# superboubek/bcd

Hardware: AMD Instinct MI355X
Metric: Mpixels/sec denoised (3-scale, b=6, w=1) (higher is better)
Workload: dtype f32

## Files before the change

bcd_amd/csrc/bcd_api.hip:

```cpp
#include "bcd_ctx.h"

#include <algorithm>
#include <chrono>
#include <climits>
#include <cmath>
#include <cstdio>
#include <cstdlib>
#include <cstring>
#include <atomic>
#include <condition_variable>
#include <mutex>
#include <new>
#include <thread>
#include <string>
#include <utility>
#include <vector>

void set_err(bcd_hip_ctx *ctx, const std::string &msg)
{
    if (!ctx) return;
    std::lock_guard<std::mutex> lock(ctx->err_mutex);
    ctx->err = msg;
}

// ... 865 lines not shown
    if (!ctx) return BCD_HIP_EINVAL;
    ctx->profiling = enabled != 0;
    return BCD_HIP_OK;
}

int bcd_hip_set_concurrent_scales(bcd_hip_ctx *ctx, int enabled)
{
    if (!ctx) return BCD_HIP_EINVAL;
    ctx->concurrent_scales = enabled != 0;
    return BCD_HIP_OK;
}

int bcd_hip_set_strict_eigensolver(int enabled)
{
    bcd_bayes27_set_strict_eigensolver(enabled);
    return BCD_HIP_OK;
}

int bcd_hip_set_fast_similarity(bcd_hip_ctx *ctx, int enabled)
{
    if (!ctx) return BCD_HIP_EINVAL;
    ctx->fast_similarity = enabled != 0;
    return BCD_HIP_OK;
}

int bcd_hip_set_cu_share(bcd_hip_ctx *ctx, int percent)
{
    if (!ctx || percent < 1 || percent > 100) return BCD_HIP_EINVAL;
    ctx->cu_share_pct = percent;
    return BCD_HIP_OK;
// ... 892 lines not shown
```

bcd_amd/csrc/bcd_launch.h:

```cpp
#pragma once
#include "bcd_common.h"

#include <stddef.h>

size_t bcd_pairdist_lds_bytes(int D, int b);
hipError_t bcd_launch_pairdist(const float *hist, const float *ns, int W, int H, int D, int b, float *T, uint8_t *Cn, int fast, int *d_range_flag, float uni_n,
                               hipStream_t st);
hipError_t bcd_launch_uniform_n(const float *ns, int64_t npix, int *d_out, hipStream_t st);
hipError_t bcd_launch_compare_planes(const float *Ta, const uint8_t *Ca, const float *Tb, const uint8_t *Cb, int64_t n, unsigned long long *out, hipStream_t st);
hipError_t bcd_launch_selftest_div(uint32_t seed, int blocks, int per_thread, unsigned long long *d_mismatches, hipStream_t st);
hipError_t bcd_launch_masks(const float *T, const uint8_t *Cn, int W, int H, int w, int b, float tau, uint32_t *mask, int32_t *count, uint32_t *fwd_scratch,
                            hipStream_t st, const BcdBorderline *ap, const float *hist, const float *ns, int D);
hipError_t bcd_launch_masks_finish(int W, int H, int b, float tau, uint32_t *mask, int32_t *count, uint32_t *fwd_scratch, hipStream_t st, const BcdBorderline *ap,
                                   const float *hist, const float *ns, int D);
hipError_t bcd_launch_window_distances(const float *T, const uint8_t *Cn, int W, int H, int w, int b, int r, int c, float *out, hipStream_t st);

hipError_t bcd_launch_pairdist_moments(const float *colors, const float *pixcov, int W, int H, int b, float var_floor, float *T, uint8_t *Cn, hipStream_t st);

hipError_t bcd_pairdist_guide_launchable(int F, int has_var, int b);
hipError_t bcd_launch_pairdist_guide(const float *features, const float *variances, int F, const float *floors, int W, int H, int b, float *T, uint8_t *Cn,
                                     hipStream_t st);
hipError_t bcd_launch_gate_masks(uint32_t *mask, const uint32_t *gate, int32_t *nsim, int W, int H, int b, hipStream_t st);
hipError_t bcd_launch_scale_inplace(float *x, float a, int64_t n, hipStream_t st);

// ... 61 lines not shown

size_t bcd_bayes_lds_bytes(int w, int b);
size_t bcd_bayes_scratch_bytes_per_block(int w, int b);
hipError_t bcd_launch_bayes_strong(const float *colors, const float *pixcov, const uint32_t *mask, const int32_t *list, const int32_t *d_nlist, int *d_work, int blocks,
                                   int W, int H, int w, int b, float min_eig, float *sum, int32_t *cnt, float *gscratch, size_t gscratch_bytes, hipStream_t st);
hipError_t bcd_launch_bayes_weak(const float *colors, const uint32_t *mask, const int32_t *list, const int32_t *d_nlist, int blocks, int W, int H, int w, int b,
                                 float *sum, int32_t *cnt, hipStream_t st);
hipError_t bcd_launch_bayes_weak_tiles(const float *colors, const uint32_t *mask, const uint8_t *state, const int32_t *nsim, int min_strong, int W, int H, int b,
                                       float *sum, int32_t *cnt, hipStream_t st, int row_begin, int row_end, const long long *skip_if);
hipError_t bcd_launch_bayes_weak_tiles_layers(const BcdLayerTable &t, int layers, const uint32_t *mask, const uint8_t *state, const int32_t *nsim, int min_strong,
                                              int W, int H, int b, hipStream_t st, int row_begin, int row_end);

size_t bcd_bayes27_record_bytes();
void bcd_bayes27_set_strict_eigensolver(int on);
float bcd_bayes27_conv2(int strict);
hipError_t bcd_launch_jacobi27_batch(const float *A, int n, int *d_work, int blocks, float *eig, float *V, hipStream_t st, float conv2 = 1e-12f, float *Aout = nullptr,
                                     const int *d_n = nullptr, int first_item = 0);
hipError_t bcd_launch_bayes27(const float *colors, const float *pixcov, const uint32_t *mask, const int32_t *list, int first_item, int nb_items, int *d_work,
                              int num_cus, int W, int H, int b, float min_eig, float *records, float *sum, int32_t *cnt, int *d_spectral, hipStream_t st,
                              int defer_redo, const int *d_nb_items);
hipError_t bcd_launch_bayes27_redo(const float *colors, const float *pixcov, const uint32_t *mask, const int32_t *list, int first_item, int nb_items, int *d_work,
                                   int num_cus, int W, int H, int b, float min_eig, float *records, float *sum, int32_t *cnt, hipStream_t st);

size_t bcd_accum_snapshot_lds(int D);
hipError_t bcd_launch_accum_dense(const float *samples, const float *weights, int64_t p0, int64_t npix, int64_t N, int k, int channels, int nbins, float gamma,
                                  float maxval, float *st, hipStream_t s);
hipError_t bcd_launch_accum_dense_layers(const BcdAccumLayerIn &in, int nb_layers, const float *weights, int64_t p0, int64_t npix, int64_t N, int k, int channels,
                                         float *layers, hipStream_t s);
hipError_t bcd_launch_accum_segments_layers(const uint32_t *keys, const uint32_t *vals, int64_t n, int64_t N, const BcdAccumLayerIn &in, int nb_layers,
                                            const float *weights, float *layers, hipStream_t s);
// ... 23 lines not shown
```

bcd_amd/csrc/bcd_selftest.hip:

```cpp
#include "bcd_ctx.h"

#include <algorithm>
#include <cstring>

namespace {

struct DevAlloc {
    void *p = nullptr;
    DevAlloc() = default;
    DevAlloc(const DevAlloc &) = delete;
    DevAlloc &operator=(const DevAlloc &) = delete;
    ~DevAlloc() { if (p) (void)hipFree(p); }
};

}

extern "C" {

int bcd_hip_selftest_distance_kernels(bcd_hip_ctx *ctx, const float *d_hist, const float *d_ns, int W, int H, int D, int search_radius,
                                      int *variant, int64_t *mismatches)
{
    if (!ctx || !d_hist || !d_ns || !mismatches || W <= 0 || H <= 0 || D <= 0 || search_radius < 1) return bad(ctx, "bad argument");
    DEVICE_GUARD(ctx);
    touch(ctx->main);
// ... 142 lines not shown
    DEVICE_GUARD(ctx);
    touch(ctx->main);
    Work &wk = ctx->main;
    RCCHK(ensure(ctx, wk.counters, sizeof(Counters)));
    RCCHK(ensure(ctx, wk.work_q, BCD_WORK_INTS * sizeof(int32_t)));
    int32_t *d_c = (int32_t *)wk.work_q.p;
    HIPCHK(ctx, hipMemsetAsync(d_c, 0, BCD_WORK_INTS * sizeof(int32_t), wk.stream));
    HIPCHK(ctx, hipEventRecord(wk.ev_stage[0], wk.stream));
    HIPCHK(ctx, bcd_launch_jacobi27_batch(d_A, n, d_c, std::min(ctx->num_cus * 12, (n + 1) / 2), d_eig, d_V, wk.stream, bcd_bayes27_conv2(production_rule ? 0 : 1)));
    HIPCHK(ctx, hipEventRecord(wk.ev_stage[1], wk.stream));
    HIPCHK(ctx, hipStreamSynchronize(wk.stream));
    if (ms) *ms = stage_ms(wk, 0, 1);
    return BCD_HIP_OK;
}

int bcd_hip_selftest_division(bcd_hip_ctx *ctx, uint32_t seed, int64_t samples, int64_t *mismatches)
{
    if (!ctx || !mismatches || samples <= 0) return bad(ctx, "bad argument");
    DEVICE_GUARD(ctx);
    touch(ctx->main);
    RCCHK(ensure(ctx, ctx->main.counters, sizeof(Counters)));
    unsigned long long *d = &ctx->main.d_counters()->selftest.result;
    HIPCHK(ctx, hipMemsetAsync(d, 0, sizeof(unsigned long long), ctx->stream));
    const int per_thread = 1024, blocks = (int)std::min<int64_t>(1 << 20, (samples + 256ll * per_thread - 1) / (256ll * per_thread));
    HIPCHK(ctx, bcd_launch_selftest_div(seed, blocks, per_thread, d, ctx->stream));
    unsigned long long h = 0;
    HIPCHK(ctx, hipMemcpyAsync(&h, d, sizeof(h), hipMemcpyDeviceToHost, ctx->stream));
    HIPCHK(ctx, hipStreamSynchronize(ctx->stream));
    *mismatches = (int64_t)h;
    return BCD_HIP_OK;
// ... 117 lines not shown
```

bcd_amd/csrc/k_bayes27.hip:

```cpp
#include "bcd_common.h"
#include <atomic>
#include <cstdio>
#include <algorithm>
#include <cstdlib>

namespace {


constexpr int K = 27, KP = 28, LD = 29, P = 9, MSZ = KP * KP, CHUNK = MSZ / K;

typedef float v16f __attribute__((ext_vector_type(16)));

struct Geom27 {
    int W, H, b, side, words, maxS;
};

#define LDS_POINTER(p) __builtin_assume(__builtin_amdgcn_is_shared((const __attribute__((address_space(0))) void *)(p)))

__device__ inline float pos_phi(float di, float dj)
{
    const float hi = fmaxf(di, dj), lo = fminf(di, dj);
    if (lo > 0.f) return 1.f;
    if (hi <= 0.f) return 0.f;
    return hi * __builtin_amdgcn_rcpf(hi - lo);
// ... 392 lines not shown
            float out[JLD], vout[JLD];
#pragma unroll
            for (int k = 0; k < JLD; ++k) { out[YSTEP ? JSY[k] : JSX[k]] = row[k]; vout[YSTEP ? JSY[k] : JSX[k]] = vrow[k]; }
#pragma unroll
            for (int k = 0; k < JLD; ++k) vrow[k] = vout[k];
            if (isRow) {
#pragma unroll
                for (int q4 = 0; q4 < JLD / 4; ++q4)
                    reinterpret_cast<float4 *>(dst)[q4] = make_float4(out[4 * q4], out[4 * q4 + 1], out[4 * q4 + 2], out[4 * q4 + 3]);
            }
        }
        wave_sync();
        __builtin_amdgcn_sched_barrier(0);
}

__global__ __launch_bounds__(64, 3) void k_jacobi27_quads(const float *Ain, int n, int *work, float *__restrict__ eig,
                                                          float *__restrict__ Vout, float conv2, float *Aout, const int *d_n, int first_item)
{
    n = items_on_device(d_n, first_item, n);
    __shared__ float4 lds4[(2 * JQ_HALF + 32) / 4];
    float *lds = reinterpret_cast<float *>(lds4);
    int *place_tab = reinterpret_cast<int *>(lds + 2 * JQ_HALF);
    const int lane = threadIdx.x, h = lane >> 5, r = lane & 31;
    const bool isRow = r < KP;
    if (lane < KP) place_tab[lane] = JPLACE[lane];
    float *Ah = lds + h * JQ_HALF, *dv_h = Ah + JQ_MAT, *rot_h = dv_h + 32;
    const int rr_ = isRow ? r : JIDLE_ROW;
    const int sx = isRow ? JSX[rr_] : 0, sy = isRow ? JSY[rr_] : 0;
    float *src = Ah + JPLACE[rr_];
    float *dst_x = Ah + JPLACE[sx], *dst_y = Ah + JPLACE[sy];
    const float *wsrc = src + (isRow ? (r & ~3) : 0);
    const int me = r & 3;
    wave_sync();
    WorkCursor cursor = work_begin();
    for (;;) {
        const int pair = work_next(work, (n + 1) / 2, lane, cursor);
        if (pair < 0) break;
        const int first = 2 * pair;
        const int item = first + h;
        const bool live = item < n;
        {
            const float4 *gsrc = reinterpret_cast<const float4 *>(Ain + (size_t)(live ? item : first) * (KP * JLD));
            for (int e = r; e < KP * JLD / 4; e += 32) {
                float4 v = gsrc[e];
                const int e0 = 4 * e, rr = e0 / JLD, c0 = e0 - rr * JLD;
                if (!live) v = make_float4(rr == c0, rr == c0 + 1, rr == c0 + 2, rr == c0 + 3);
                *reinterpret_cast<float4 *>(Ah + place_tab[rr] + c0) = v;
            }
            if (isRow) dv_h[r] = 1.f;
        }
        wave_sync();
        float vrow[JLD];
// ... 48 lines not shown
            if (isRow) eig[(size_t)item * KP + r] = src[r];
        }
        if (Aout) {
            if (isRow) rot_h[r] = src[r];
            wave_sync();
            if (isRow && live) jacobi_write_correction(Aout + (size_t)item * (KP * JLD) + r * JLD, src, rot_h, r);
        }
        if (live) {
            if (r < K) {
                float4 *o = reinterpret_cast<float4 *>(Vout + (size_t)item * (KP * JLD) + r * JLD);
#pragma unroll
                for (int q4 = 0; q4 < JLD / 4; ++q4) o[q4] = make_float4(vrow[4 * q4], vrow[4 * q4 + 1], vrow[4 * q4 + 2], vrow[4 * q4 + 3]);
            }
        }
        wave_sync();
    }
}

__device__ void add_noise27(float *M, const float *noise, int lane, float sign)
{
    for (int t = lane; t < P * 9; t += 64) {
        int blk = t / 9, e = t - blk * 9, i = e / 3, j = e - i * 3;
        M[(3 * blk + i) * LD + 3 * blk + j] += sign * noise[blk * 6 + noise_idx(i, j)];
    }
    __syncthreads();
}


__device__ inline float bcast_lane(float v, int k) { return __int_as_float(__builtin_amdgcn_readlane(__float_as_int(v), k)); }

// ... 730 lines not shown
    for (int t = lane; t < P * 9; t += 64) {
        const int ro = t / 9, ij = t - 9 * ro, i = ij / 3, j = ij - 3 * i;
        float *e = tile + (3 * ro + i) * LD + 3 * ro + j;
        *e -= noise[ro * 6 + noise_idx(i, j)];
    }
    for (int e = lane; e < KP * (JLD / 4); e += 64) {
        const int r = e / (JLD / 4), q = e - r * (JLD / 4);
        const float *src = tile + r * LD + 4 * q;
        reinterpret_cast<float4 *>(recA)[e] = make_float4(src[0], src[1], src[2], src[3]);
    }
    const bool poisoned = noise_poisons_item(noise, lane);
    if (lane < P * 6) recX[lane] = noise[lane];
    if (lane < K) recX[P * 6 + lane] = poisoned ? __builtin_nanf("") : mean[lane];
}

template <int PHASE, int B = WB>
__global__ __launch_bounds__(64, PHASE == 1 ? 5 : 3) void k_bayes27w(const float *__restrict__ colors, const float *__restrict__ pixcov,
                                                 const uint32_t *__restrict__ mask, const int32_t *__restrict__ list,
                                                 int first_item, int nb_items, int *work, Geom27 g, float min_eig, Records27 rec, float *sum,
                                                 int32_t *cnt, const int *redo ,
                                                 const int *d_n = nullptr)
{
    extern __shared__ float lds[];
    const int lane = threadIdx.x;
    nb_items = items_on_device(d_n, first_item, nb_items);
    if (PHASE == 2 && redo) nb_items = redo[0];
    if (PHASE == 1 && redo && blockIdx.x == 0 && lane == 0) const_cast<int *>(redo)[0] = 0;
    float *Cm = lds, *A = Cm + MSZ, *V = A + MSZ, *Bm = V + MSZ;
    float *cwin = PHASE == 1 ? lds : Bm;
    static_assert(PHASE == 1 || B == WB, "the LDS finish (PHASE 2) exists for the default search radius only");
    float *nwin = cwin + W1L<B>::NWIN;
    float *cs = Bm + MSZ;
    float *noise = PHASE == 1 ? lds + W1L<B>::NOISE : cs + 2 * KP;
    float *mean = noise + 56;
    float *fl = mean + KP;
    uint16_t *mem = reinterpret_cast<uint16_t *>(PHASE == 1 ? lds + W1L<B>::MEM : fl + KP);
    static_assert(WPIX * 3 <= MSZ, "the colour window fits a matrix buffer");
    for (int e = lane; e < (PHASE == 1 ? W1L<B>::MEM_SLOTS : WinT<B>::MEM); e += 64) mem[e] = (uint16_t)((WinT<B>::AW + 1) * (PHASE == 1 ? 3 : 1));
    if (lane == 0) mean[K] = 0.f;
    __syncthreads();
    const int W = g.W, H = g.H;

  WorkCursor cursor = work_begin();
  for (;;) {
    int slot = work_next(work, nb_items, lane, cursor);
    if (slot < 0) break;
    if (PHASE == 2 && redo) slot = __builtin_amdgcn_readfirstlane(redo[1 + slot]);
    const int p = __builtin_amdgcn_readfirstlane(list[first_item + slot]);
    const int pr = p / W, pc = p - pr * W;
    float *recA = rec.A + (size_t)slot * MSZ, *recC = rec.C + (size_t)slot * MSZ, *recX = rec.aux + (size_t)slot * AUX27;

  if (PHASE == 1) {
    const int n = win_stage_phase1<B>(cwin, nwin, mem, colors, pixcov, mask, p, pr, pc, W, H, g.words, lane);
    win_noise_mean<B>(noise, mean, cwin, nwin, mem, n, lane, pixcov, (pr - (B + 1)) * W + pc - (B + 1), W);
    win_covariance<B>(nwin , cwin, mean, mem, n, lane);
    win_write_records(recA, recC, recX, nwin, noise, mean, lane);
    __syncthreads();
  } else {
    const int n = decode_members_win<WB>(mask, p, g.words, mem, lane);
    {
        const float *recV = rec.V + (size_t)slot * MSZ;
        for (int e = lane; e < MSZ / 4; e += 64) {
            reinterpret_cast<float4 *>(Cm)[e] = reinterpret_cast<const float4 *>(recC)[e];
            reinterpret_cast<float4 *>(V)[e] = reinterpret_cast<const float4 *>(recV)[e];
        }
        if (lane < P * 6) noise[lane] = recX[lane];
        if (lane < K) mean[lane] = recX[P * 6 + lane];
        if (lane < KP) fl[lane] = fmaxf(0.f, rec.eig[(size_t)slot * KP + lane]);
        __syncthreads();
    }
    pos_part_lds(Bm, A, fl, V, recA, rec.eig + (size_t)slot * KP, lane);
// ... 79 lines not shown
    {
        constexpr int row3 = WAW * 3;
        const long long base = (long long)p - (long long)(WB + 1) * W - (WB + 1);
        for (int e = lane; e < WAW * row3; e += 64) {
            int wy = e / row3, r = e - wy * row3, wx = r / 3;
            if (accC[wy * WAW + wx] != 0) unsafeAtomicAdd(sum + (base + (long long)wy * W) * 3 + r, accS[e]);
        }
        for (int e = lane; e < WPIX; e += 64) {
            int wy = e / WAW, wx = e - wy * WAW, c = accC[e];
            if (c != 0 && cnt) atomicAdd(cnt + (base + (long long)wy * W + wx), c);
        }
    }
    __syncthreads();
  }
  }
}

template <int B>
__global__ __launch_bounds__(64, 3) void k_finish27w(const float *__restrict__ colors, const uint32_t *__restrict__ mask,
                                                     const int32_t *__restrict__ list, int first_item, int nb_items, int *work, Geom27 g,
                                                     float min_eig, Records27 rec, float *sum, int32_t *cnt, int *redo ,
                                                     int *redo_total , const int *d_n)
{
    nb_items = items_on_device(d_n, first_item, nb_items);
    using G_ = WinT<B>;
    constexpr int AW = G_::AW, PIX = G_::PIX, GAP = G_::G;
    extern __shared__ float lds[];
    const int lane0 = threadIdx.x;
    float *cwin = lds, *accS = lds + G_::F2_ACCS;
    int *accC = reinterpret_cast<int *>(lds + G_::F2_ACCC);
// ... 197 lines not shown

hipError_t bcd_launch_jacobi27_batch(const float *A, int n, int *d_work, int blocks, float *eig, float *V, hipStream_t st, float conv2 = 1e-12f, float *Aout = nullptr,
                                     const int *d_n = nullptr, int first_item = 0);

static std::atomic<int> g_strict_eigen{ -1 };
void bcd_bayes27_set_strict_eigensolver(int on) { g_strict_eigen.store(on ? 1 : 0); }
static float jacobi_conv2()
{
    int v = g_strict_eigen.load();
    if (v < 0) { const char *e = getenv("BCD_HIP_STRICT_EIGEN"); v = (e && e[0] == '1') ? 1 : 0; g_strict_eigen.store(v); }
    return v ? JACOBI_CONV2_STRICT : JACOBI_CONV2_CORRECTED;
}

float bcd_bayes27_conv2(int strict) { return strict ? JACOBI_CONV2_STRICT : JACOBI_CONV2_CORRECTED; }

hipError_t bcd_launch_bayes27(const float *colors, const float *pixcov, const uint32_t *mask, const int32_t *list, int first_item, int nb_items,
                              int *d_work, int num_cus, int W, int H, int b, float min_eig, float *records, float *sum,
                              int32_t *cnt, int *d_spectral , hipStream_t st,
                              int defer_redo ,
                              const int *d_nb_items )
{
    const int *dn = d_nb_items;
    if (nb_items <= 0) return hipSuccess;
    Geom27 g;
    g.W = W; g.H = H; g.b = b; g.side = 2 * b + 1; g.words = (g.side * g.side + 31) / 32; g.maxS = g.side * g.side;
    if (g.words > 32) return hipErrorInvalidValue;
    Records27 rec;
    rec.A = records;
    rec.V = rec.A + (size_t)nb_items * MSZ;
    rec.C = rec.V + (size_t)nb_items * MSZ;
    rec.aux = rec.C + (size_t)nb_items * MSZ;
    rec.eig = rec.aux + (size_t)nb_items * AUX27;
    const size_t lds2 = bcd_bayes27_lds_bytes(b), lds1 = lds2 - 3 * MSZ * sizeof(float);
    const int per_cu1 = (int)std::min<size_t>(20, (size_t)160 * 1024 / lds1), per_cu2 = (int)std::min<size_t>(12, (size_t)160 * 1024 / lds2);
    if (b == WB) {
        const size_t wl1 = W1L<WB>::BYTES;
        const size_t wl2 = (size_t)W2_MEM * sizeof(float) + WMEM * sizeof(uint16_t);
        const int w_cu1 = (int)std::min<size_t>(20, (size_t)160 * 1024 / wl1), w_cu2 = (int)std::min<size_t>(12, (size_t)160 * 1024 / wl2);
        static const bool lds_algebra = [] { const char *e = getenv("BCD_HIP_FINISH_LDS"); return e && e[0] == '1'; }();
        int *redo = reinterpret_cast<int *>(rec.eig + (size_t)nb_items * KP);
        hipLaunchKernelGGL(k_bayes27w<1>, dim3(std::min(nb_items, num_cus * w_cu1)), dim3(64), wl1, st, colors, pixcov, mask, list, first_item, nb_items,
                           d_work, g, min_eig, rec, sum, cnt, lds_algebra ? nullptr : redo, dn);
        { hipError_t e = bcd_launch_jacobi27_batch(rec.A, nb_items, d_work + BCD_WORK_QUEUES * BCD_WORK_STRIDE, std::min((nb_items + 1) / 2, num_cus * 12), rec.eig, rec.V, st, jacobi_conv2(), rec.A, dn, first_item); if (e != hipSuccess) return e; }
        if (lds_algebra)
            hipLaunchKernelGGL(k_bayes27w<2>, dim3(std::min(nb_items, num_cus * w_cu2)), dim3(64), wl2, st, colors, pixcov, mask, list, first_item, nb_items,
                               d_work + 2 * BCD_WORK_QUEUES * BCD_WORK_STRIDE, g, min_eig, rec, sum, cnt, nullptr, dn);
        else {
            const size_t wl3 = WinT<WB>::F2_BYTES;
            hipLaunchKernelGGL(k_finish27w<WB>, dim3(std::min(nb_items, num_cus * 12)), dim3(64), wl3, st, colors, mask, list, first_item, nb_items,
                               d_work + 2 * BCD_WORK_QUEUES * BCD_WORK_STRIDE, g, min_eig, rec, sum, cnt, redo, d_spectral, dn);
            if (!defer_redo)
                hipLaunchKernelGGL(k_bayes27w<2>, dim3(std::min(nb_items, num_cus * 2)), dim3(64), wl2, st, colors, pixcov, mask, list, first_item, nb_items,
                                   d_work + 3 * BCD_WORK_QUEUES * BCD_WORK_STRIDE, g, min_eig, rec, sum, cnt, redo, dn);
        }
        return hipGetLastError();
    }
    constexpr int WB2 = 12;
    static const bool finish_lds_b12 = [] { const char *e = getenv("BCD_HIP_FINISH_LDS"); return e && e[0] == '1'; }();
// ... 55 lines not shown
    const size_t wl2 = (size_t)W2_MEM * sizeof(float) + WMEM * sizeof(uint16_t);
    hipLaunchKernelGGL(k_bayes27w<2>, dim3(std::min(nb_items, num_cus * 2)), dim3(64), wl2, st, colors, pixcov, mask, list, first_item, nb_items,
                       d_work + 3 * BCD_WORK_QUEUES * BCD_WORK_STRIDE, g, min_eig, rec, sum, cnt, redo);
    return hipGetLastError();
}

hipError_t bcd_launch_jacobi27_batch(const float *A, int n, int *d_work, int blocks, float *eig, float *V, hipStream_t st, float conv2, float *Aout,
                                     const int *d_n , int first_item)
{
    if (blocks <= 0) return hipSuccess;
    static const bool pairs = [] { const char *e = getenv("BCD_HIP_JACOBI_PAIRS"); return e && e[0] == '1'; }();
    if (pairs) hipLaunchKernelGGL((k_jacobi27_batch<true, true>), dim3(blocks), dim3(64), 0, st, A, n, d_work, eig, V, 1e-12f, Aout, d_n, first_item);
    else hipLaunchKernelGGL(k_jacobi27_quads, dim3(blocks), dim3(64), 0, st, A, n, d_work, eig, V, conv2, Aout, d_n, first_item);
    return hipGetLastError();
}
```

bcd_amd/hip.py:

```python
import ctypes as C
import os
import weakref

_HERE = os.path.dirname(os.path.abspath(__file__))
LIB_PATH = os.environ.get("BCD_HIP_LIB") or os.path.join(_HERE, "lib", "libbcd_hip.so")

_F = C.POINTER(C.c_float)
_VP = C.c_void_p


class Params(C.Structure):
    _fields_ = [("hist_dist_threshold", C.c_float), ("patch_radius", C.c_int32), ("search_radius", C.c_int32),
                ("min_eigen_value", C.c_float), ("use_random_pixel_order", C.c_int32),
                ("marked_skip_probability", C.c_float), ("order_seed", C.c_uint32)]


MAX_LAYERS = 16


class Layer(C.Structure):
    _fields_ = [("d_colors", C.c_void_p), ("d_covariances", C.c_void_p), ("d_out", C.c_void_p)]


class SelectionScale(C.Structure):
# ... 184 lines not shown
    return out


PROGRESS_FN = C.CFUNCTYPE(None, C.c_float, C.c_void_p)


class ScaleStats(C.Structure):
    _fields_ = [("width", C.c_int32), ("height", C.c_int32), ("main_pixels", C.c_int64), ("processed", C.c_int64),
                ("fallback", C.c_int64), ("similar_total", C.c_int64), ("active_rounds", C.c_int32),
                ("ms_similarity", C.c_float), ("ms_active", C.c_float), ("ms_bayes", C.c_float), ("ms_total", C.c_float),
                ("similarity_path", C.c_int32), ("borderline_pairs", C.c_int32), ("cu_share", C.c_int32), ("spectral_inverses", C.c_int32)]


SYMBOLS = [
    "bcd_hip_ctx_create", "bcd_hip_ctx_destroy", "bcd_hip_last_error", "bcd_hip_device_count", "bcd_hip_default_params",
    "bcd_hip_set_profiling", "bcd_hip_set_concurrent_scales", "bcd_hip_set_fast_similarity", "bcd_hip_set_strict_eigensolver", "bcd_hip_set_cu_share", "bcd_hip_get_stats", "bcd_hip_kernel_time", "bcd_hip_reset_kernel_time",
    "bcd_hip_denoise", "bcd_hip_denoise_layers", "bcd_hip_denoise_layers_host", "bcd_hip_denoise_layers_host_ex",
    "bcd_hip_spike_map", "bcd_hip_spike_apply", "bcd_hip_spike_filter_layers",
    "bcd_hip_similarity_masks_moments", "bcd_hip_window_distances_moments", "bcd_hip_denoise_moments", "bcd_hip_denoise_moments_host",
    "bcd_hip_similarity_masks_guide", "bcd_hip_window_distances_guide", "bcd_hip_gate_masks", "bcd_hip_denoise_guided", "bcd_hip_denoise_guided_host",
    "bcd_hip_selection_create", "bcd_hip_selection_destroy", "bcd_hip_denoise_layers_keep", "bcd_hip_selection_denoise", "bcd_hip_selection_info", "bcd_hip_selection_read",
    "bcd_hip_accum_moments", "bcd_hip_layer_spectral_inverses", "bcd_hip_denoise_begin", "bcd_hip_denoise_wait", "bcd_hip_denoise_band", "bcd_hip_denoise_bands", "bcd_hip_denoise_host", "bcd_hip_denoise_host_ex", "bcd_hip_last_upload_bytes", "bcd_hip_selftest_pack32", "bcd_hip_set_progress_callback",
    "bcd_hip_multi_create", "bcd_hip_multi_destroy", "bcd_hip_multi_last_error", "bcd_hip_multi_get_stats", "bcd_hip_multi_set_progress_callback", "bcd_hip_multi_set_frame_timeout", "bcd_hip_multi_set_comm_trace", "bcd_hip_multi_get_comm_trace", "bcd_hip_multi_denoise_host",
    "bcd_hip_multi_unique_id", "bcd_hip_multi_rccl_info", "bcd_hip_multi_create_rank", "bcd_hip_multi_rank_configure", "bcd_hip_multi_rank_upload", "bcd_hip_multi_rank_step",
    "bcd_hip_multi_rank_download", "bcd_hip_multi_rank_renew_ids", "bcd_hip_multi_set_loopback", "bcd_hip_multi_selftest_transport",
    "bcd_hip_scale_begin", "bcd_hip_pixel_cov", "bcd_hip_similarity_masks", "bcd_hip_similarity_masks_deferred", "bcd_hip_similarity_masks_verdict", "bcd_hip_similarity_masks_exact", "bcd_hip_similarity_last_path", "bcd_hip_window_distances", "bcd_hip_active_set", "bcd_hip_active_init", "bcd_hip_active_step", "bcd_hip_active_step_enqueue", "bcd_hip_active_step_collect",
    "bcd_hip_bayes_accumulate", "bcd_hip_bayes_accumulate_layers", "bcd_hip_layers_pixel_cov", "bcd_hip_layers_finalize", "bcd_hip_layers_downscale_avg", "bcd_hip_layers_downscale_cov", "bcd_hip_layers_merge",
    "bcd_hip_bayes_accumulate_rows", "bcd_hip_bayes_last_redo_count", "bcd_hip_finalize", "bcd_hip_finalize_band", "bcd_hip_downscale_sum", "bcd_hip_downscale_avg",
    "bcd_hip_downscale_cov", "bcd_hip_interpolate", "bcd_hip_merge", "bcd_hip_spike_filter", "bcd_hip_accumulate_samples", "bcd_hip_accum_create", "bcd_hip_accum_destroy", "bcd_hip_accum_reset", "bcd_hip_accum_add_dense",
    "bcd_hip_accum_add_scattered", "bcd_hip_accum_statistics", "bcd_hip_accum_info", "bcd_hip_default_plan_params", "bcd_hip_accum_plan", "bcd_hip_zero_bad_values",
    "bcd_hip_accum_set_filter", "bcd_hip_accum_add_splatted", "bcd_hip_filter_table",
    "bcd_hip_accum_state_info", "bcd_hip_accum_state_bytes", "bcd_hip_accum_export", "bcd_hip_accum_import", "bcd_hip_accum_merge_state", "bcd_hip_accum_merge",
    "bcd_hip_accum_create_layers", "bcd_hip_accum_nb_layers", "bcd_hip_accum_add_dense_layers", "bcd_hip_accum_add_scattered_layers", "bcd_hip_accum_add_splatted_layers",
    "bcd_hip_accum_layer_statistics", "bcd_hip_accum_layers_state_info", "bcd_hip_accum_layers_state_bytes", "bcd_hip_accum_export_layers", "bcd_hip_accum_import_layers",
    "bcd_hip_accum_merge_layers_state",
    "bcd_hip_visit_order", "bcd_hip_scale_seed", "bcd_hip_strip_order_seed", "bcd_hip_selftest_division", "bcd_hip_selftest_distance_kernels", "bcd_hip_selftest_approx_distance", "bcd_hip_selftest_bin_work", "bcd_hip_eig27_batch", "bcd_hip_eig27_batch_rule",
    "bcd_hip_selftest_sparse_upload", "bcd_hip_selftest_host_stream", "bcd_hip_approx_planes", "bcd_hip_selftest_active_lists",
]

_lib = None


def lib():
    global _lib
    if _lib is None:
        if not os.path.exists(LIB_PATH):
            raise RuntimeError("libbcd_hip.so is not built (%s): run `python -m bcd_amd.build`; "
                               "there is no CPU fallback" % LIB_PATH)
        _lib = C.CDLL(LIB_PATH)
        _lib.bcd_hip_last_error.restype = C.c_char_p
        _lib.bcd_hip_last_error.argtypes = [_VP]
        _lib.bcd_hip_scale_seed.restype = C.c_uint32
# ... 672 lines not shown
        H, W, D = hist.shape
        a, b_, c = C.c_int64(0), C.c_int64(0), C.c_int64(0)
        ms = C.c_float(0)
        self._chk(lib().bcd_hip_selftest_bin_work(self.h, _dp(hist), _dp(ns), W, H, D, int(b), int(reps), C.byref(a), C.byref(b_), C.byref(c), C.byref(ms)))
        return a.value, b_.value, c.value, ms.value

    def eig27_batch(self, A, production_rule=False):
        torch = self.torch
        n = A.shape[0]
        eig = torch.zeros((n, 28), dtype=torch.float32, device=A.device)
        V = torch.zeros((n, 28, 28), dtype=torch.float32, device=A.device)
        ms = C.c_float(0)
        self._chk(lib().bcd_hip_eig27_batch_rule(self.h, _dp(A), n, _dp(eig), _dp(V), C.byref(ms), 1 if production_rule else 0))
        return eig, V, ms.value

    def selftest_division(self, samples, seed=1):
        n = C.c_int64(-1)
        self._chk(lib().bcd_hip_selftest_division(self.h, C.c_uint32(seed), C.c_int64(samples), C.byref(n)))
        return n.value

    def synchronize(self):
        self.torch.cuda.synchronize(self.device)


class Accumulator:

    def __init__(self, ctx, W, H, nbins=20, gamma=2.2, maxval=2.5, capacity=0, layers=0):
        L = lib()
        L.bcd_hip_accum_create.argtypes = [_VP, C.c_int, C.c_int, C.c_int, C.c_float, C.c_float, C.c_int64, C.POINTER(_VP)]
        L.bcd_hip_accum_destroy.argtypes = [_VP]
# ... 330 lines not shown
    def comm_trace(self, rank):
        n = lib().bcd_hip_multi_get_comm_trace(self.h, rank, None, 0)
        buf = (C.c_int64 * max(1, n))()
        n = lib().bcd_hip_multi_get_comm_trace(self.h, rank, buf, n)
        v = list(buf[:n])
        return [tuple(v[i:i + 4]) for i in range(0, n, 4)]


MULTI_ID_BYTES = 128


def set_strict_eigensolver(on):
    lib().bcd_hip_set_strict_eigensolver(1 if on else 0)


def rccl_info():
    buf = C.create_string_buffer(512)
    lib().bcd_hip_multi_rccl_info(buf, 512)
    mapped = []
    try:
        for ln in open("/proc/self/maps"):
            f = ln.split()
            if len(f) >= 6 and "librccl" in f[5] and f[5] not in mapped:
                mapped.append(f[5])
    except OSError:
        pass
    native = buf.value.decode()
    path = native.split(" from ", 1)[1] if " from " in native else "?"
    return {"native": native, "mapped": mapped, "one_copy": len(mapped) <= 1, "native_is_mapped": os.path.realpath(path) in [os.path.realpath(m) for m in mapped]}

# ... 97 lines not shown
```

include/bcd_hip.h:

```cpp
#ifndef BCD_HIP_H
#define BCD_HIP_H

#include <stdint.h>

#ifdef __cplusplus
extern "C" {
#endif

#define BCD_HIP_OK 0
#define BCD_HIP_EINVAL (-1)
#define BCD_HIP_EDEVICE (-2)
#define BCD_HIP_ENOMEM (-3)
#define BCD_HIP_EUNSUPPORTED (-4)

typedef struct bcd_hip_ctx bcd_hip_ctx;

typedef void (*bcd_hip_progress_fn)(float progress, void *user);

typedef struct bcd_hip_params {
    float    hist_dist_threshold;
    int32_t  patch_radius;
    int32_t  search_radius;
    float    min_eigen_value;
    int32_t  use_random_pixel_order;
// ... 15 lines not shown
    int32_t similarity_path;
    int32_t borderline_pairs;
    int32_t cu_share;
    int32_t spectral_inverses;
} bcd_hip_scale_stats;

int  bcd_hip_ctx_create(bcd_hip_ctx **ctx, int device, void *hip_stream );
void bcd_hip_ctx_destroy(bcd_hip_ctx *ctx);
const char *bcd_hip_last_error(const bcd_hip_ctx *ctx);
int  bcd_hip_device_count(void);
void bcd_hip_default_params(bcd_hip_params *p);
int  bcd_hip_set_profiling(bcd_hip_ctx *ctx, int enabled);
int  bcd_hip_set_concurrent_scales(bcd_hip_ctx *ctx, int enabled);
int  bcd_hip_set_fast_similarity(bcd_hip_ctx *ctx, int enabled);
int  bcd_hip_set_strict_eigensolver(int enabled);
int  bcd_hip_set_cu_share(bcd_hip_ctx *ctx, int percent);
int  bcd_hip_set_progress_callback(bcd_hip_ctx *ctx, bcd_hip_progress_fn fn, void *user);
int  bcd_hip_get_stats(const bcd_hip_ctx *ctx, int scale, bcd_hip_scale_stats *out);
int  bcd_hip_kernel_time(const bcd_hip_ctx *ctx, float *ms_pairdist, int32_t *launches);
int  bcd_hip_reset_kernel_time(bcd_hip_ctx *ctx);

int bcd_hip_denoise(bcd_hip_ctx *ctx, const float *d_colors, const float *d_nsamples,
                    const float *d_histograms, const float *d_covariances,
                    int W, int H, int D, int nb_scales, const bcd_hip_params *prm, float *d_out);

int bcd_hip_denoise_begin(bcd_hip_ctx *ctx, const float *d_colors, const float *d_nsamples,
                          const float *d_histograms, const float *d_covariances,
                          int W, int H, int D, int nb_scales, const bcd_hip_params *prm, float *d_out);
int bcd_hip_denoise_wait(bcd_hip_ctx *ctx);

// ... 295 lines not shown
    int32_t chunks_done;
    int32_t range_flag;
    float   uni_n;
    int32_t ratio_form;
} bcd_hip_host_stream_result;
int bcd_hip_selftest_host_stream(bcd_hip_ctx *ctx, const float *h_colors, const float *h_nsamples, const float *h_histograms, const float *h_covariances,
                                 int W, int H, int D, const bcd_hip_params *prm, float spike_factor, int stop_after_chunks, int poison,
                                 void *d_planes, uint8_t *d_counts, float *d_colors_out, float *d_nsamples_out, float *d_histograms_out,
                                 float *d_covariances_out, float *d_hist_uploaded, bcd_hip_host_stream_result *res);
int bcd_hip_approx_planes(bcd_hip_ctx *ctx, const float *d_hist, const float *d_nsamples, int W, int H, int D, int search_radius, float uni_n,
                          int ratio_form, float tau, void *d_planes, uint8_t *d_counts, int *range_flag);

int bcd_hip_eig27_batch(bcd_hip_ctx *ctx, const float *d_A, int n, float *d_eig, float *d_V, float *ms);
int bcd_hip_eig27_batch_rule(bcd_hip_ctx *ctx, const float *d_A, int n, float *d_eig, float *d_V, float *ms, int production_rule);

int bcd_hip_visit_order(int W, int H, int patch_radius, int random_order, uint32_t seed, int32_t *h_order);
uint32_t bcd_hip_strip_order_seed(int W, int H, int patch_radius, int search_radius);
uint32_t bcd_hip_scale_seed(uint32_t seed0, int scale);

#ifdef __cplusplus
}
#endif
#endif
```

Before: 473.8.

## Fuse window preparation and 27x27 Jacobi eigensolve into one kernel

Adds a kernel that, per work-queue pair, builds the covariance records for two pixels in LDS and then runs the Jacobi quad eigensolver on them in the same workgroup, overlaying the solver's LDS area on the window buffers. This replaces the separate prepare kernel plus jacobi batch launch by default, removing one launch and the round trip of matrices through global memory between them. The fused kernel runs at lower occupancy (launch bounds 3 and the larger window LDS), and it serialises two preparations before each solve. An environment switch and a selftest compare the fused and split paths bit-for-bit.

Measured after the change: 486.0 (median of 6 runs). 1.03x the previous value.

```diff
diff --git a/bcd_amd/csrc/bcd_api.hip b/bcd_amd/csrc/bcd_api.hip
--- a/bcd_amd/csrc/bcd_api.hip
+++ b/bcd_amd/csrc/bcd_api.hip
@@ -903,6 +903,12 @@
 int bcd_hip_set_strict_eigensolver(int enabled)
 {
     bcd_bayes27_set_strict_eigensolver(enabled);
+    return BCD_HIP_OK;
+}
+
+int bcd_hip_set_fused_prepare_solve(int enabled)
+{
+    bcd_bayes27_set_fused_prepare_solve(enabled);
     return BCD_HIP_OK;
 }
 
diff --git a/bcd_amd/csrc/bcd_launch.h b/bcd_amd/csrc/bcd_launch.h
--- a/bcd_amd/csrc/bcd_launch.h
+++ b/bcd_amd/csrc/bcd_launch.h
@@ -99,6 +99,11 @@
 size_t bcd_bayes27_record_bytes();
 void bcd_bayes27_set_strict_eigensolver(int on);
 float bcd_bayes27_conv2(int strict);
+void bcd_bayes27_set_fused_prepare_solve(int on);
+int bcd_bayes27_fused_prepare_solve();
+hipError_t bcd_launch_prepare_solve27(const float *colors, const float *pixcov, const uint32_t *mask, const int32_t *list, int first_item, int nb_items,
+                                      int *d_work, int num_cus, int W, int H, float *records, hipStream_t st, const int *d_nb_items, int fused);
+hipError_t bcd_launch_count_differing_words(const void *a, const void *b, size_t words, unsigned long long *d_count, hipStream_t st);
 hipError_t bcd_launch_jacobi27_batch(const float *A, int n, int *d_work, int blocks, float *eig, float *V, hipStream_t st, float conv2 = 1e-12f, float *Aout = nullptr,
                                      const int *d_n = nullptr, int first_item = 0);
 hipError_t bcd_launch_bayes27(const float *colors, const float *pixcov, const uint32_t *mask, const int32_t *list, int first_item, int nb_items, int *d_work,
diff --git a/bcd_amd/csrc/bcd_selftest.hip b/bcd_amd/csrc/bcd_selftest.hip
--- a/bcd_amd/csrc/bcd_selftest.hip
+++ b/bcd_amd/csrc/bcd_selftest.hip
@@ -180,6 +180,41 @@
     return BCD_HIP_OK;
 }
 
+int bcd_hip_selftest_prepare_solve(bcd_hip_ctx *ctx, const float *d_colors, const float *d_pixcov, const uint32_t *d_mask, const int32_t *d_list,
+                                   int capacity, int list_len, int W, int H, int search_radius, int cu_share_pct, int64_t *differing_words)
+{
+    if (!ctx || !d_colors || !d_pixcov || !d_mask || !d_list || !differing_words || capacity <= 0 || W < 3 || H < 3) return bad(ctx, "bad argument");
+    if (search_radius != 6) { set_err(ctx, "the fused kernel serves search radius 6"); return BCD_HIP_EUNSUPPORTED; }
+    if (cu_share_pct < 1 || cu_share_pct > 100) return bad(ctx, "bad CU share");
+    DEVICE_GUARD(ctx);
+    touch(ctx->main);
+    Work &wk = ctx->main;
+    RCCHK(ensure(ctx, wk.counters, sizeof(Counters)));
+    RCCHK(ensure(ctx, wk.work_q, BCD_WORK_INTS * sizeof(int32_t)));
+    const size_t bytes = bcd_bayes27_record_bytes() * (size_t)capacity;
+    const size_t words = (bytes - 2 * sizeof(int) * (size_t)capacity) / 4 + 1;
+    DevAlloc rec[2], len;
+    for (int i = 0; i < 2; ++i)
+        if (hipMalloc(&rec[i].p, bytes) != hipSuccess) { set_err(ctx, "hipMalloc"); return BCD_HIP_ENOMEM; }
+    HIPCHK(ctx, hipMalloc(&len.p, sizeof(int)));
+    const int cus = std::max(1, ctx->num_cus * cu_share_pct / 100);
+    unsigned long long *d_cnt = &wk.d_counters()->selftest.result;
+    HIPCHK(ctx, hipMemsetAsync(d_cnt, 0, sizeof(*d_cnt), wk.stream));
+    if (list_len >= 0) HIPCHK(ctx, hipMemcpyAsync(len.p, &list_len, sizeof(int), hipMemcpyHostToDevice, wk.stream));
+    for (int fused = 0; fused < 2; ++fused) {
+        HIPCHK(ctx, hipMemsetAsync(rec[fused].p, 0xA5, bytes, wk.stream));
+        HIPCHK(ctx, hipMemsetAsync(wk.work_q.p, 0, BCD_WORK_INTS * sizeof(int32_t), wk.stream));
+        HIPCHK(ctx, bcd_launch_prepare_solve27(d_colors, d_pixcov, d_mask, d_list, 0, capacity, (int *)wk.work_q.p, cus, W, H, (float *)rec[fused].p, wk.stream,
+                                               list_len >= 0 ? (const int *)len.p : nullptr, fused));
+    }
+    HIPCHK(ctx, bcd_launch_count_differing_words(rec[0].p, rec[1].p, words, d_cnt, wk.stream));
+    unsigned long long h = 0;
+    HIPCHK(ctx, hipMemcpyAsync(&h, d_cnt, sizeof(h), hipMemcpyDeviceToHost, wk.stream));
+    HIPCHK(ctx, hipStreamSynchronize(wk.stream));
+    *differing_words = (int64_t)h;
+    return BCD_HIP_OK;
+}
+
 int bcd_hip_selftest_division(bcd_hip_ctx *ctx, uint32_t seed, int64_t samples, int64_t *mismatches)
 {
     if (!ctx || !mismatches || samples <= 0) return bad(ctx, "bad argument");
diff --git a/bcd_amd/csrc/k_bayes27.hip b/bcd_amd/csrc/k_bayes27.hip
--- a/bcd_amd/csrc/k_bayes27.hip
+++ b/bcd_amd/csrc/k_bayes27.hip
@@ -430,28 +430,41 @@
         __builtin_amdgcn_sched_barrier(0);
 }
 
-__global__ __launch_bounds__(64, 3) void k_jacobi27_quads(const float *Ain, int n, int *work, float *__restrict__ eig,
-                                                          float *__restrict__ Vout, float conv2, float *Aout, const int *d_n, int first_item)
-{
-    n = items_on_device(d_n, first_item, n);
-    __shared__ float4 lds4[(2 * JQ_HALF + 32) / 4];
-    float *lds = reinterpret_cast<float *>(lds4);
+struct JqLane {
+    float *Ah, *dv_h, *rot_h, *src, *dst_x, *dst_y;
+    const float *wsrc;
+    const int *place_tab;
+    int h, r, me, sx, sy;
+    bool isRow;
+};
+constexpr int JQ_LDS = 2 * JQ_HALF + 32;
+
+__device__ __forceinline__ JqLane jq_lane_setup(float *lds, int lane)
+{
+    JqLane L;
     int *place_tab = reinterpret_cast<int *>(lds + 2 * JQ_HALF);
-    const int lane = threadIdx.x, h = lane >> 5, r = lane & 31;
-    const bool isRow = r < KP;
+    L.place_tab = place_tab;
+    L.h = lane >> 5; L.r = lane & 31;
+    L.isRow = L.r < KP;
     if (lane < KP) place_tab[lane] = JPLACE[lane];
-    float *Ah = lds + h * JQ_HALF, *dv_h = Ah + JQ_MAT, *rot_h = dv_h + 32;
-    const int rr_ = isRow ? r : JIDLE_ROW;
-    const int sx = isRow ? JSX[rr_] : 0, sy = isRow ? JSY[rr_] : 0;
-    float *src = Ah + JPLACE[rr_];
-    float *dst_x = Ah + JPLACE[sx], *dst_y = Ah + JPLACE[sy];
-    const float *wsrc = src + (isRow ? (r & ~3) : 0);
-    const int me = r & 3;
-    wave_sync();
-    WorkCursor cursor = work_begin();
-    for (;;) {
-        const int pair = work_next(work, (n + 1) / 2, lane, cursor);
-        if (pair < 0) break;
+    L.Ah = lds + L.h * JQ_HALF; L.dv_h = L.Ah + JQ_MAT; L.rot_h = L.dv_h + 32;
+    const int rr_ = L.isRow ? L.r : JIDLE_ROW;
+    L.sx = L.isRow ? JSX[rr_] : 0; L.sy = L.isRow ? JSY[rr_] : 0;
+    L.src = L.Ah + JPLACE[rr_];
+    L.dst_x = L.Ah + JPLACE[L.sx]; L.dst_y = L.Ah + JPLACE[L.sy];
+    L.wsrc = L.src + (L.isRow ? (L.r & ~3) : 0);
+    L.me = L.r & 3;
+    return L;
+}
+
+__device__ __forceinline__ void jacobi_quads_pair(const JqLane &L, int pair, int n, const float *Ain, float *__restrict__ eig, float *__restrict__ Vout,
+                                                  float conv2, float *Aout)
+{
+        const int h = L.h, r = L.r, me = L.me, sx = L.sx, sy = L.sy;
+        const bool isRow = L.isRow;
+        float *Ah = L.Ah, *dv_h = L.dv_h, *rot_h = L.rot_h, *src = L.src, *dst_x = L.dst_x, *dst_y = L.dst_y;
+        const float *wsrc = L.wsrc;
+        const int *place_tab = L.place_tab;
         const int first = 2 * pair;
         const int item = first + h;
         const bool live = item < n;
@@ -530,6 +543,21 @@
             }
         }
         wave_sync();
+}
+
+__global__ __launch_bounds__(64, 3) void k_jacobi27_quads(const float *Ain, int n, int *work, float *__restrict__ eig,
+                                                          float *__restrict__ Vout, float conv2, float *Aout, const int *d_n, int first_item)
+{
+    n = items_on_device(d_n, first_item, n);
+    __shared__ float4 lds4[JQ_LDS / 4];
+    const int lane = threadIdx.x;
+    const JqLane L = jq_lane_setup(reinterpret_cast<float *>(lds4), lane);
+    wave_sync();
+    WorkCursor cursor = work_begin();
+    for (;;) {
+        const int pair = work_next(work, (n + 1) / 2, lane, cursor);
+        if (pair < 0) break;
+        jacobi_quads_pair(L, pair, n, Ain, eig, Vout, conv2, Aout);
     }
 }
 
@@ -1290,6 +1318,33 @@
     if (lane < K) recX[P * 6 + lane] = poisoned ? __builtin_nanf("") : mean[lane];
 }
 
+template <int B>
+__device__ __forceinline__ void win_prepare_lds_init(float *lds, int lane)
+{
+    uint16_t *mem = reinterpret_cast<uint16_t *>(lds + W1L<B>::MEM);
+    float *mean = lds + W1L<B>::NOISE + 56;
+    for (int e = lane; e < W1L<B>::MEM_SLOTS; e += 64) mem[e] = (uint16_t)((WinT<B>::AW + 1) * 3);
+    if (lane == 0) mean[K] = 0.f;
+    __syncthreads();
+}
+
+template <int B>
+__device__ __forceinline__ void win_prepare_item(float *lds, int slot, const float *__restrict__ colors, const float *__restrict__ pixcov,
+                                                 const uint32_t *__restrict__ mask, const int32_t *__restrict__ list, int first_item, const Geom27 &g,
+                                                 const Records27 &rec, int lane)
+{
+    float *cwin = lds, *nwin = cwin + W1L<B>::NWIN, *noise = lds + W1L<B>::NOISE, *mean = noise + 56;
+    uint16_t *mem = reinterpret_cast<uint16_t *>(lds + W1L<B>::MEM);
+    const int W = g.W, H = g.H;
+    const int p = __builtin_amdgcn_readfirstlane(list[first_item + slot]);
+    const int pr = p / W, pc = p - pr * W;
+    float *recA = rec.A + (size_t)slot * MSZ, *recC = rec.C + (size_t)slot * MSZ, *recX = rec.aux + (size_t)slot * AUX27;
+    const int n = win_stage_phase1<B>(cwin, nwin, mem, colors, pixcov, mask, p, pr, pc, W, H, g.words, lane);
+    win_noise_mean<B>(noise, mean, cwin, nwin, mem, n, lane, pixcov, (pr - (B + 1)) * W + pc - (B + 1), W);
+    win_covariance<B>(nwin , cwin, mean, mem, n, lane);
+    win_write_records(recA, recC, recX, nwin, noise, mean, lane);
+}
+
 template <int PHASE, int B = WB>
 __global__ __launch_bounds__(64, PHASE == 1 ? 5 : 3) void k_bayes27w(const float *__restrict__ colors, const float *__restrict__ pixcov,
                                                  const uint32_t *__restrict__ mask, const int32_t *__restrict__ list,
@@ -1312,9 +1367,12 @@
     float *fl = mean + KP;
     uint16_t *mem = reinterpret_cast<uint16_t *>(PHASE == 1 ? lds + W1L<B>::MEM : fl + KP);
     static_assert(WPIX * 3 <= MSZ, "the colour window fits a matrix buffer");
-    for (int e = lane; e < (PHASE == 1 ? W1L<B>::MEM_SLOTS : WinT<B>::MEM); e += 64) mem[e] = (uint16_t)((WinT<B>::AW + 1) * (PHASE == 1 ? 3 : 1));
-    if (lane == 0) mean[K] = 0.f;
-    __syncthreads();
+    if (PHASE == 1) win_prepare_lds_init<B>(lds, lane);
+    else {
+        for (int e = lane; e < WinT<B>::MEM; e += 64) mem[e] = (uint16_t)(WinT<B>::AW + 1);
+        if (lane == 0) mean[K] = 0.f;
+        __syncthreads();
+    }
     const int W = g.W, H = g.H;
 
   WorkCursor cursor = work_begin();
@@ -1327,10 +1385,7 @@
     float *recA = rec.A + (size_t)slot * MSZ, *recC = rec.C + (size_t)slot * MSZ, *recX = rec.aux + (size_t)slot * AUX27;
 
   if (PHASE == 1) {
-    const int n = win_stage_phase1<B>(cwin, nwin, mem, colors, pixcov, mask, p, pr, pc, W, H, g.words, lane);
-    win_noise_mean<B>(noise, mean, cwin, nwin, mem, n, lane, pixcov, (pr - (B + 1)) * W + pc - (B + 1), W);
-    win_covariance<B>(nwin , cwin, mean, mem, n, lane);
-    win_write_records(recA, recC, recX, nwin, noise, mean, lane);
+    win_prepare_item<B>(lds, slot, colors, pixcov, mask, list, first_item, g, rec, lane);
     __syncthreads();
   } else {
     const int n = decode_members_win<WB>(mask, p, g.words, mem, lane);
@@ -1440,6 +1495,45 @@
     __syncthreads();
   }
   }
+}
+
+template <int B>
+__global__ __launch_bounds__(64, 3) void k_prepare_solve27(const float *__restrict__ colors, const float *__restrict__ pixcov,
+                                                           const uint32_t *__restrict__ mask, const int32_t *__restrict__ list, int first_item,
+                                                           int nb_items, int *work, Geom27 g, Records27 rec, int *redo ,
+                                                           float conv2, const int *d_n)
+{
+    static_assert(W1L<B>::COV_WINDOW, "the default search radius");
+    static_assert(JQ_LDS <= W1L<B>::NOISE && JQ_LDS * sizeof(float) <= W1L<B>::BYTES, "the solver's area overlays the windows only");
+    extern __shared__ float lds[];
+    const int lane0 = threadIdx.x;
+    const int n = items_on_device(d_n, first_item, nb_items);
+    if (redo && blockIdx.x == 0 && lane0 == 0) redo[0] = 0;
+    win_prepare_lds_init<B>(lds, lane0);
+    WorkCursor cursor = work_begin();
+    for (;;) {
+        const int pair = work_next(work, (n + 1) / 2, lane0, cursor);
+        if (pair < 0) break;
+        win_prepare_item<B>(lds, 2 * pair, colors, pixcov, mask, list, first_item, g, rec, lane0);
+        if (2 * pair + 1 < n) {
+            __syncthreads();
+            win_prepare_item<B>(lds, 2 * pair + 1, colors, pixcov, mask, list, first_item, g, rec, lane0);
+        }
+        __syncthreads();
+        __builtin_amdgcn_fence(__ATOMIC_SEQ_CST, "workgroup");
+        int lane = lane0;
+        asm volatile("" : "+v"(lane));
+        const JqLane L = jq_lane_setup(lds, lane);
+        wave_sync();
+        jacobi_quads_pair(L, pair, n, rec.A, rec.eig, rec.V, conv2, rec.A);
+    }
+}
+
+__global__ void k_count_differing_words(const uint32_t *__restrict__ a, const uint32_t *__restrict__ b, size_t words, unsigned long long *count)
+{
+    unsigned int mine = 0;
+    for (size_t i = (size_t)blockIdx.x * blockDim.x + threadIdx.x; i < words; i += (size_t)gridDim.x * blockDim.x) mine += a[i] != b[i];
+    if (mine) atomicAdd(count, (unsigned long long)mine);
 }
 
 template <int B>
@@ -1667,6 +1761,32 @@
 
 float bcd_bayes27_conv2(int strict) { return strict ? JACOBI_CONV2_STRICT : JACOBI_CONV2_CORRECTED; }
 
+static std::atomic<int> g_fused_prepare_solve{ -1 };
+void bcd_bayes27_set_fused_prepare_solve(int on) { g_fused_prepare_solve.store(on ? 1 : 0); }
+int bcd_bayes27_fused_prepare_solve()
+{
+    int v = g_fused_prepare_solve.load();
+    if (v < 0) { const char *e = getenv("BCD_HIP_PREPARE_SOLVE_SPLIT"); v = (e && e[0] == '1') ? 0 : 1; g_fused_prepare_solve.store(v); }
+    return v;
+}
+
+static hipError_t launch_prepare_solve27(const float *colors, const float *pixcov, const uint32_t *mask, const int32_t *list, int first_item, int nb_items,
+                                         int *d_work, int num_cus, const Geom27 &g, const Records27 &rec, int *redo, hipStream_t st, const int *dn, int fused)
+{
+    static const bool pairs = [] { const char *e = getenv("BCD_HIP_JACOBI_PAIRS"); return e && e[0] == '1'; }();
+    const size_t wl1 = W1L<WB>::BYTES;
+    if (fused && !pairs) {
+        hipLaunchKernelGGL(k_prepare_solve27<WB>, dim3(std::min((nb_items + 1) / 2, num_cus * 12)), dim3(64), wl1, st, colors, pixcov, mask, list, first_item,
+                           nb_items, d_work, g, rec, redo, jacobi_conv2(), dn);
+        return hipGetLastError();
+    }
+    const int w_cu1 = (int)std::min<size_t>(20, (size_t)160 * 1024 / wl1);
+    hipLaunchKernelGGL(k_bayes27w<1>, dim3(std::min(nb_items, num_cus * w_cu1)), dim3(64), wl1, st, colors, pixcov, mask, list, first_item, nb_items,
+                       d_work, g, 0.f, rec, (float *)nullptr, (int32_t *)nullptr, (const int *)redo, dn);
+    return bcd_launch_jacobi27_batch(rec.A, nb_items, d_work + BCD_WORK_QUEUES * BCD_WORK_STRIDE, std::min((nb_items + 1) / 2, num_cus * 12), rec.eig, rec.V, st,
+                                     jacobi_conv2(), rec.A, dn, first_item);
+}
+
 hipError_t bcd_launch_bayes27(const float *colors, const float *pixcov, const uint32_t *mask, const int32_t *list, int first_item, int nb_items,
                               int *d_work, int num_cus, int W, int H, int b, float min_eig, float *records, float *sum,
                               int32_t *cnt, int *d_spectral , hipStream_t st,
@@ -1687,14 +1807,12 @@
     const size_t lds2 = bcd_bayes27_lds_bytes(b), lds1 = lds2 - 3 * MSZ * sizeof(float);
     const int per_cu1 = (int)std::min<size_t>(20, (size_t)160 * 1024 / lds1), per_cu2 = (int)std::min<size_t>(12, (size_t)160 * 1024 / lds2);
     if (b == WB) {
-        const size_t wl1 = W1L<WB>::BYTES;
         const size_t wl2 = (size_t)W2_MEM * sizeof(float) + WMEM * sizeof(uint16_t);
-        const int w_cu1 = (int)std::min<size_t>(20, (size_t)160 * 1024 / wl1), w_cu2 = (int)std::min<size_t>(12, (size_t)160 * 1024 / wl2);
+        const int w_cu2 = (int)std::min<size_t>(12, (size_t)160 * 1024 / wl2);
         static const bool lds_algebra = [] { const char *e = getenv("BCD_HIP_FINISH_LDS"); return e && e[0] == '1'; }();
         int *redo = reinterpret_cast<int *>(rec.eig + (size_t)nb_items * KP);
-        hipLaunchKernelGGL(k_bayes27w<1>, dim3(std::min(nb_items, num_cus * w_cu1)), dim3(64), wl1, st, colors, pixcov, mask, list, first_item, nb_items,
-                           d_work, g, min_eig, rec, sum, cnt, lds_algebra ? nullptr : redo, dn);
-        { hipError_t e = bcd_launch_jacobi27_batch(rec.A, nb_items, d_work + BCD_WORK_QUEUES * BCD_WORK_STRIDE, std::min((nb_items + 1) / 2, num_cus * 12), rec.eig, rec.V, st, jacobi_conv2(), rec.A, dn, first_item); if (e != hipSuccess) return e; }
+        { hipError_t e = launch_prepare_solve27(colors, pixcov, mask, list, first_item, nb_items, d_work, num_cus, g, rec, lds_algebra ? nullptr : redo, st, dn,
+                                                bcd_bayes27_fused_prepare_solve()); if (e != hipSuccess) return e; }
         if (lds_algebra)
             hipLaunchKernelGGL(k_bayes27w<2>, dim3(std::min(nb_items, num_cus * w_cu2)), dim3(64), wl2, st, colors, pixcov, mask, list, first_item, nb_items,
                                d_work + 2 * BCD_WORK_QUEUES * BCD_WORK_STRIDE, g, min_eig, rec, sum, cnt, nullptr, dn);
@@ -1780,3 +1898,27 @@
     else hipLaunchKernelGGL(k_jacobi27_quads, dim3(blocks), dim3(64), 0, st, A, n, d_work, eig, V, conv2, Aout, d_n, first_item);
     return hipGetLastError();
 }
+
+hipError_t bcd_launch_prepare_solve27(const float *colors, const float *pixcov, const uint32_t *mask, const int32_t *list, int first_item, int nb_items,
+                                      int *d_work, int num_cus, int W, int H, float *records, hipStream_t st, const int *d_nb_items, int fused)
+{
+    if (nb_items <= 0) return hipSuccess;
+    Geom27 g;
+    g.W = W; g.H = H; g.b = WB; g.side = 2 * WB + 1; g.words = (g.side * g.side + 31) / 32; g.maxS = g.side * g.side;
+    Records27 rec;
+    rec.A = records;
+    rec.V = rec.A + (size_t)nb_items * MSZ;
+    rec.C = rec.V + (size_t)nb_items * MSZ;
+    rec.aux = rec.C + (size_t)nb_items * MSZ;
+    rec.eig = rec.aux + (size_t)nb_items * AUX27;
+    int *redo = reinterpret_cast<int *>(rec.eig + (size_t)nb_items * KP);
+    return launch_prepare_solve27(colors, pixcov, mask, list, first_item, nb_items, d_work, num_cus, g, rec, redo, st, d_nb_items, fused);
+}
+
+hipError_t bcd_launch_count_differing_words(const void *a, const void *b, size_t words, unsigned long long *d_count, hipStream_t st)
+{
+    if (words == 0) return hipSuccess;
+    const int blocks = (int)std::min<size_t>(1024, (words + 255) / 256);
+    hipLaunchKernelGGL(k_count_differing_words, dim3(blocks), dim3(256), 0, st, (const uint32_t *)a, (const uint32_t *)b, words, d_count);
+    return hipGetLastError();
+}
diff --git a/bcd_amd/hip.py b/bcd_amd/hip.py
--- a/bcd_amd/hip.py
+++ b/bcd_amd/hip.py
@@ -222,7 +222,7 @@
 
 SYMBOLS = [
     "bcd_hip_ctx_create", "bcd_hip_ctx_destroy", "bcd_hip_last_error", "bcd_hip_device_count", "bcd_hip_default_params",
-    "bcd_hip_set_profiling", "bcd_hip_set_concurrent_scales", "bcd_hip_set_fast_similarity", "bcd_hip_set_strict_eigensolver", "bcd_hip_set_cu_share", "bcd_hip_get_stats", "bcd_hip_kernel_time", "bcd_hip_reset_kernel_time",
+    "bcd_hip_set_profiling", "bcd_hip_set_concurrent_scales", "bcd_hip_set_fast_similarity", "bcd_hip_set_strict_eigensolver", "bcd_hip_set_fused_prepare_solve", "bcd_hip_set_cu_share", "bcd_hip_get_stats", "bcd_hip_kernel_time", "bcd_hip_reset_kernel_time",
     "bcd_hip_denoise", "bcd_hip_denoise_layers", "bcd_hip_denoise_layers_host", "bcd_hip_denoise_layers_host_ex",
     "bcd_hip_spike_map", "bcd_hip_spike_apply", "bcd_hip_spike_filter_layers",
     "bcd_hip_similarity_masks_moments", "bcd_hip_window_distances_moments", "bcd_hip_denoise_moments", "bcd_hip_denoise_moments_host",
@@ -243,7 +243,7 @@
     "bcd_hip_accum_layer_statistics", "bcd_hip_accum_layers_state_info", "bcd_hip_accum_layers_state_bytes", "bcd_hip_accum_export_layers", "bcd_hip_accum_import_layers",
     "bcd_hip_accum_merge_layers_state",
     "bcd_hip_visit_order", "bcd_hip_scale_seed", "bcd_hip_strip_order_seed", "bcd_hip_selftest_division", "bcd_hip_selftest_distance_kernels", "bcd_hip_selftest_approx_distance", "bcd_hip_selftest_bin_work", "bcd_hip_eig27_batch", "bcd_hip_eig27_batch_rule",
-    "bcd_hip_selftest_sparse_upload", "bcd_hip_selftest_host_stream", "bcd_hip_approx_planes", "bcd_hip_selftest_active_lists",
+    "bcd_hip_selftest_sparse_upload", "bcd_hip_selftest_host_stream", "bcd_hip_approx_planes", "bcd_hip_selftest_active_lists", "bcd_hip_selftest_prepare_solve",
 ]
 
 _lib = None
@@ -946,6 +946,16 @@
         self._chk(lib().bcd_hip_eig27_batch_rule(self.h, _dp(A), n, _dp(eig), _dp(V), C.byref(ms), 1 if production_rule else 0))
         return eig, V, ms.value
 
+    def selftest_prepare_solve(self, col, pixcov, mask, items, capacity=None, list_len=None, b=6, cu_share_pct=100):
+        H, W, _ = col.shape
+        cap = int(items.numel() if capacity is None else capacity)
+        assert mask.shape[0] == H and mask.shape[1] == W and pixcov.shape[:2] == col.shape[:2]
+        assert min(cap, cap if list_len is None else int(list_len)) <= items.numel()
+        n = C.c_int64(-1)
+        self._chk(lib().bcd_hip_selftest_prepare_solve(self.h, _dp(col), _dp(pixcov), _dp(mask), _dp(items), cap, -1 if list_len is None else int(list_len),
+                                                       W, H, int(b), int(cu_share_pct), C.byref(n)))
+        return n.value
+
     def selftest_division(self, samples, seed=1):
         n = C.c_int64(-1)
         self._chk(lib().bcd_hip_selftest_division(self.h, C.c_uint32(seed), C.c_int64(samples), C.byref(n)))
@@ -1306,6 +1316,10 @@
     lib().bcd_hip_set_strict_eigensolver(1 if on else 0)
 
 
+def set_fused_prepare_solve(on):
+    lib().bcd_hip_set_fused_prepare_solve(1 if on else 0)
+
+
 def rccl_info():
     buf = C.create_string_buffer(512)
     lib().bcd_hip_multi_rccl_info(buf, 512)
diff --git a/include/bcd_hip.h b/include/bcd_hip.h
--- a/include/bcd_hip.h
+++ b/include/bcd_hip.h
@@ -53,6 +53,7 @@
 int  bcd_hip_set_concurrent_scales(bcd_hip_ctx *ctx, int enabled);
 int  bcd_hip_set_fast_similarity(bcd_hip_ctx *ctx, int enabled);
 int  bcd_hip_set_strict_eigensolver(int enabled);
+int  bcd_hip_set_fused_prepare_solve(int enabled);
 int  bcd_hip_set_cu_share(bcd_hip_ctx *ctx, int percent);
 int  bcd_hip_set_progress_callback(bcd_hip_ctx *ctx, bcd_hip_progress_fn fn, void *user);
 int  bcd_hip_get_stats(const bcd_hip_ctx *ctx, int scale, bcd_hip_scale_stats *out);
@@ -378,6 +379,9 @@
 int bcd_hip_eig27_batch(bcd_hip_ctx *ctx, const float *d_A, int n, float *d_eig, float *d_V, float *ms);
 int bcd_hip_eig27_batch_rule(bcd_hip_ctx *ctx, const float *d_A, int n, float *d_eig, float *d_V, float *ms, int production_rule);
 
+int bcd_hip_selftest_prepare_solve(bcd_hip_ctx *ctx, const float *d_colors, const float *d_pixcov, const uint32_t *d_mask, const int32_t *d_list,
+                                   int capacity, int list_len, int W, int H, int search_radius, int cu_share_pct, int64_t *differing_words);
+
 int bcd_hip_visit_order(int W, int H, int patch_radius, int random_order, uint32_t seed, int32_t *h_order);
 uint32_t bcd_hip_strip_order_seed(int W, int H, int patch_radius, int search_radius);
 uint32_t bcd_hip_scale_seed(uint32_t seed0, int scale);
```
